# chronista-club/fleetflow

Hardware: AMD Instinct MI355X
Metric: container x node evaluations/sec (FFD what-if plans, work-equivalent) + achieved GB/s % HBM roofline (higher is better)
Workload: dtype u32

## Files before the change

### fleetflow_amd/csrc/fp_internal.h

```cpp
#pragma once
#include <cmath>
#include <cstring>
#include <hip/hip_runtime.h>
#include <stdint.h>
#include <vector>
#include "../../include/fleetplace.h"
#include "fp_rows.h"

#define FP_HIP(call)                                   \
    do {                                               \
        hipError_t e_ = (call);                        \
        if (e_ != hipSuccess) return fp_hip_fail(e_);  \
    } while (0)

int fp_hip_fail(hipError_t e);

__device__ __forceinline__ void fp_or_new_bits(uint32_t *w, uint32_t bits) {
    if (bits & ~*(volatile uint32_t *)w) atomicOr(w, bits);
}

struct fp_ctx {
    int device = 0;
    hipStream_t own_stream = nullptr;
    hipStream_t stream = nullptr;
// ... 115 lines not shown
    const double r = pow((double)hi / (double)lo, 1.0 / (double)(FP_BUCKETS - 2));
    double v = (double)lo;
    for (int k = 1; k < FP_BUCKETS; ++k) {
        uint32_t x = k == FP_BUCKETS - 1 ? hi : (uint32_t)ceil(v);
        if (x < T[k - 1]) x = T[k - 1];
        if (x > hi) x = hi;
        T[k] = x;
        v *= r;
    }
}
struct fp_pipe_soa {
    uint32_t *s_cpu, *s_mem, *s_req, *s_conf, *s_idx;
};
int fp_pipe_soa_take(fp_ctx *c, size_t SC, fp_pipe_soa *soa);
uint32_t fp_pipe_kpack(const fp_ctx *c, uint32_t C);
int fp_pipe_launch(fp_ctx *c, uint32_t S, uint32_t C, uint32_t N, uint32_t scen_base, const uint32_t *order,
                   const void *skeys, uint32_t key_bytes, uint32_t mbits, uint64_t cmax, uint64_t mmax,
                   const uint32_t *cval, const uint32_t *mval, const fp_batch *b, const uint32_t *thr,
                   const fp_pipe_soa *ready, uint32_t *rng);

namespace fpd {

constexpr uint64_t GAMMA = 0x9E3779B97F4A7C15ull;
constexpr uint64_t TAG_CONT = 0xC0C0C0C0C0C0C0C0ull;
constexpr uint64_t TAG_NODE = 0x5E5E5E5E5E5E5E5Eull;

__host__ __device__ inline uint64_t draw(uint64_t seed, uint64_t idx) {
    uint64_t z = seed + (idx + 1) * GAMMA;
    z = (z ^ (z >> 30)) * 0xBF58476D1CE4E5B9ull;
    z = (z ^ (z >> 27)) * 0x94D049BB133111EBull;
    return z ^ (z >> 31);
// ... 18 lines not shown
```

### fleetflow_amd/csrc/fp_pipe.hip

```cpp
#include "fp_internal.h"
#include "fp_pipe_asm.h"
#include "fp_pipe_sys.h"
#include "fp_pipe_pk.h"
#include "fp_pipe_tus.h"
#include <stdlib.h>
#include <string.h>
#include <mutex>
#include <type_traits>
#include <utility>

#ifdef FP_PIPE_STATS
__device__ unsigned long long g_pipe_stats[16 * 16];
#define STAT_ADD(w, i, v) atomicAdd(&g_pipe_stats[(w) * 16 + (i)], (unsigned long long)(v))
#define STAT_CLK() __builtin_amdgcn_s_memtime()
#define STAT_ON 1
#ifdef FP_PIPE_STATS_FINE
#define STAT_GCLK() __builtin_amdgcn_s_memtime()
#define STAT_FINE 1
#else
#define STAT_GCLK() 0ull
#define STAT_FINE 0
#endif
constexpr int TL_B = 2048;
__device__ unsigned long long g_pipe_tl[16 * TL_B * 8];
// ... 33 lines not shown
    uint32_t flush;
    uint32_t kpack;
    uint32_t publish;
    uint32_t pub_mask;
    uint32_t sys;
    uint32_t *ticket;
    uint32_t *gabort;
    uint32_t *ghead;
    uint32_t *gdata;
    uint32_t *part;
    const uint32_t *s_cpu, *s_mem, *s_req, *s_conf, *s_idx;
    uint32_t *cf, *mf;
    const uint32_t *lab;
    uint32_t *cu;
    const uint8_t *sched;
    uint32_t *assign;
    uint8_t *reason;
    uint64_t *cost;
    uint32_t *err;
    uint64_t spin_ticks;
    const uint32_t *thr;
    uint32_t prio;
    uint32_t *rng;
    uint32_t pk_mode;
};

__device__ __forceinline__ uint32_t lds_acq(uint32_t *p) {
    return __builtin_amdgcn_readfirstlane(__hip_atomic_load(p, __ATOMIC_ACQUIRE, __HIP_MEMORY_SCOPE_WORKGROUP));
}
__device__ __forceinline__ void lds_rel(uint32_t *p, uint32_t v) {
    __hip_atomic_store(p, v, __ATOMIC_RELEASE, __HIP_MEMORY_SCOPE_WORKGROUP);
}

__device__ __forceinline__ uint32_t g_ld(const uint32_t *p) {
    return __hip_atomic_load(const_cast<uint32_t *>(p), __ATOMIC_RELAXED, __HIP_MEMORY_SCOPE_AGENT);
}
__device__ __forceinline__ uint32_t g_ld_u(const uint32_t *p) {
    return __builtin_amdgcn_readfirstlane(g_ld(p));
}
__device__ __forceinline__ void g_st(uint32_t *p, uint32_t v) {
// ... 501 lines not shown
                req = valid ? nf_req : 0u;
                conf = valid ? nf_conf : 0u;
                idx = valid ? nf_idx : 0u;
            } else {
                if (valid) {
                    cpu = a.s_cpu[cb + i];
                    mem = a.s_mem[cb + i];
                    req = a.s_req[cb + i];
                    conf = a.s_conf[cb + i];
                    idx = a.s_idx[cb + i];
                }
                if constexpr (DB) __builtin_amdgcn_s_waitcnt(VMCNT0);
            }
            const bool cyc = valid && (idx & CYC);
            if (cyc) {
                const uint32_t j = idx & pmask;
                a.assign[cb + j] = FP_NONE;
                a.reason[cb + j] = (uint8_t)req;
            }
            n_rej += (uint32_t)__popcll(__ballot(cyc));
            valid = valid && !cyc;
            k0 += 64;
            if constexpr (LA >= 2) {
                if (k0 < C) {
                    const size_t ti = cb + min(k0 + (lane == 0 ? 0u : lane == 1 ? 32u : 63u), C - 1);
                    g_touch(a.s_cpu + ti);
                    g_touch(a.s_mem + ti);
                    g_touch(a.s_req + ti);
                    g_touch(a.s_conf + ti);
                    g_touch(a.s_idx + ti);
                }
            }
        } else {
// ... 123 lines not shown
#ifdef FP_PIPE_STATS
        const unsigned long long tl_cand = ck_b;
        const uint32_t tl_idx = st_batches - 1;
#endif
        if constexpr (DB_EARLY) {
            asm volatile("" : "+v"(nf_cpu), "+v"(nf_mem), "+v"(nf_req), "+v"(nf_conf), "+v"(nf_idx), "+v"(la2_n),
                         "+v"(la2_pos));
            if (g_in) {
                nf_idx = la_pos;
                la_n = la2_n;
                la_pos = la2_pos;
            }
        } else if constexpr (DB) {
            FPP_REQUEST_NEXT();
        }
        if ((placed >> lane) & 1ull) a.assign[cb + (idx & pmask)] = my_assign;
#ifdef FP_PIPE_STATS
        if (s == 0 && lane == 0 && tl_idx < (uint32_t)TL_B && b * W + w < 16) {
            unsigned long long *tl = &g_pipe_tl[((size_t)(b * W + w) * TL_B + tl_idx) * 8];
            tl[0] = tl_top; tl[1] = tl_avail; tl[2] = ck_t0_batch; tl[3] = tl_pre; tl[4] = tl_cand;
            tl[5] = st_checks - tl_checks0; tl[6] = st_hits - tl_hits0;
            tl[7] = tl_todo | ((unsigned long long)__popcll(vm) << 32);
        }
#endif
        const bool fwd = valid && !((placed >> lane) & 1ull);
        if (g_out) {
            const uint64_t fm = __builtin_amdgcn_ballot_w64(fwd);
            const uint32_t f = (uint32_t)__popcll(fm);
            if (f) {
                const uint32_t pos = ofill + fpp_rank(fm);
                if (gbounded &&
// ... 18 lines not shown
                    ofill += f;
                }
            }
            if (tail_issued && ofill && __builtin_amdgcn_readfirstlane(tail_async) + 1u >= ohead) {
                if (lane == 0) g_st(gout_data + (size_t)GSLOT(ohead) * LSLOT, ofill);
                asm volatile("s_waitcnt vmcnt(0)" ::: "memory");
                ohead++;
                if (lane == 0) g_st(gout_head, ohead);
                ofill = 0;
                opend = 0;
            }
            if (STAT_FINE) { ck_b = STAT_GCLK(); ck_fwd += ck_b - ck_a; }
            continue;
        }
        if (!has_out) {
            if (fwd) {
                a.assign[cb + (idx & pmask)] = FP_NONE;
                a.reason[cb + (idx & pmask)] = FP_REASON_NOFIT;
            }
            n_rej += (uint32_t)__popcll(__ballot(fwd));
            continue;
        }
        const uint64_t fm = __ballot(fwd);
        const uint32_t f = (uint32_t)__popcll(fm);
        if (f) {
            const uint32_t pos = ofill + fpp_rank(fm);
            uint32_t *od = odata + (size_t)(ohead % R) * NF * 64;
            if (fwd && pos < 64) {
                od[pos] = cpu; od[64 + pos] = mem; od[128 + pos] = req; od[192 + pos] = conf; od[256 + pos] = idx;
            }
            if (ofill + f >= 64) {
                octl[2 + ohead % R] = 64;
                ohead++;
                lds_rel(&octl[0], ohead);
// ... 255 lines not shown
#pragma unroll
        for (int u = 0; u < 4; ++u) {
            const size_t i = i0 + (size_t)u * stride;
            if (i < total) {
                __builtin_nontemporal_store(cv[u], &s_cpu[i]);
                __builtin_nontemporal_store(mv[u], &s_mem[i]);
                __builtin_nontemporal_store(r[u], &s_req[i]);
                __builtin_nontemporal_store(f[u], &s_conf[i]);
                const uint32_t kb = kpack ? (bucket(T, cv[u]) << 21) | (bucket(T + K, mv[u]) << 26) : 0u;
                __builtin_nontemporal_store(pos[u] | kb | cy[u], &s_idx[i]);
            }
        }
    }
}

__global__ void k_gather_payload(uint32_t S, uint32_t C, const uint32_t *__restrict__ order,
                                 const uint32_t *__restrict__ req, const uint32_t *__restrict__ conf,
                                 const uint32_t *__restrict__ level, const uint32_t *__restrict__ summ,
                                 uint32_t *__restrict__ s_req, uint32_t *__restrict__ s_conf,
                                 uint32_t *__restrict__ s_idx) {
    const uint32_t total = S * C;
    const uint32_t lb = (gridDim.x & 7u) ? blockIdx.x : (blockIdx.x & 7u) * (gridDim.x >> 3) + (blockIdx.x >> 3);
    const uint32_t i0 = lb * 4 * blockDim.x + threadIdx.x;
    uint32_t src[4], r[4], f[4], cy[4];
#pragma unroll
    for (int u = 0; u < 4; ++u) {
        const uint32_t i = i0 + u * blockDim.x;
        if (i < total) src[u] = i - i % C + __builtin_nontemporal_load(&order[i]);
    }
#pragma unroll
    for (int u = 0; u < 4; ++u) {
        const uint32_t i = i0 + u * blockDim.x;
        if (i < total) {
            r[u] = req[src[u]];
            f[u] = conf[src[u]];
            cy[u] = (level && level[src[u]] == FP_NONE) ? CYC : 0u;
            if (cy[u]) {
                r[u] = FP_REASON_CYCLE;
            } else if (summ && screened(summ + (size_t)(i / C) * 4, r[u], f[u])) {
                cy[u] = CYC;
                r[u] = FP_REASON_NOFIT;
            }
        }
    }
#pragma unroll
    for (int u = 0; u < 4; ++u) {
        const uint32_t i = i0 + u * blockDim.x;
        if (i < total) {
            __builtin_nontemporal_store(r[u], &s_req[i]);
            __builtin_nontemporal_store(f[u], &s_conf[i]);
            if (cy[u]) s_idx[i] |= CYC;
        }
    }
}

constexpr uint32_t PL_THREADS = 1024, PL_H = 25, PL_MAX_C = PL_THREADS * PL_H * 2;
constexpr uint32_t PL_CHUNK = 18 * 1024;
__global__ __launch_bounds__(1024) void k_payload_lds(uint32_t C, const uint32_t *__restrict__ order,
                                                      const uint32_t *__restrict__ req,
                                                      const uint32_t *__restrict__ conf,
                                                      const uint32_t *__restrict__ level,
                                                      const uint32_t *__restrict__ summ,
                                                      uint32_t *__restrict__ s_req, uint32_t *__restrict__ s_conf,
                                                      uint32_t *__restrict__ s_idx) {
    extern __shared__ uint2 pl_lds2[];
    uint32_t *pl_lds = reinterpret_cast<uint32_t *>(pl_lds2);
    const uint32_t t = threadIdx.x;
    const size_t cb = (size_t)blockIdx.x * C;
    const uint32_t sm0 = summ ? summ[(size_t)blockIdx.x * 4] : 0xFFFFFFFFu;
    const uint32_t sm1 = summ ? summ[(size_t)blockIdx.x * 4 + 1] : 0u;
    for (uint32_t h = 0; h < 2; ++h) {
        const uint32_t pbase = h * PL_THREADS * PL_H + t;
        if (h * PL_THREADS * PL_H >= C) break;
        uint32_t o[PL_H];
#pragma unroll
        for (uint32_t j = 0; j < PL_H; ++j) {
            const uint32_t p = pbase + PL_THREADS * j;
            o[j] = p < C ? __builtin_nontemporal_load(&order[cb + p]) : 0xFFFFFFFFu;
        }
        uint32_t vr[PL_H], vf[PL_H];
        uint32_t cy = 0;
        if (level) {
            for (uint32_t a0 = 0; a0 < C; a0 += 2 * PL_CHUNK) {
                const uint32_t n = C - a0 < 2 * PL_CHUNK ? C - a0 : 2 * PL_CHUNK;
                __syncthreads();
#pragma unroll 4
                for (uint32_t i = t; i < n; i += PL_THREADS) pl_lds[i] = __builtin_nontemporal_load(&level[cb + a0 + i]);
                __syncthreads();
#pragma unroll
                for (uint32_t j = 0; j < PL_H; ++j) {
                    const uint32_t d = o[j] - a0;
                    if (d < n) cy |= (uint32_t)(pl_lds[d] == FP_NONE) << j;
                }
// ... 18 lines not shown
            if (p < C) {
                uint32_t r = vr[j];
                const bool c = (cy >> j) & 1u, x = ((r & ~sm0) | (vf[j] & sm1)) != 0u;
                if (c) r = FP_REASON_CYCLE;
                else if (summ && x) r = FP_REASON_NOFIT;
                __builtin_nontemporal_store(r, &s_req[cb + p]);
                __builtin_nontemporal_store(vf[j], &s_conf[cb + p]);
                if (c || (summ && x)) s_idx[cb + p] |= CYC;
            }
        }
    }
}

constexpr uint32_t UNSORT_SPAN16 = 50 * 1024;
constexpr uint32_t UNSORT_SPAN32 = 30 * 1024;
template <bool NARROW>
__global__ __launch_bounds__(1024) void k_unsort(uint32_t C, uint32_t H, uint32_t span,
                                                 const uint32_t *__restrict__ order,
                                                 const uint32_t *__restrict__ asg_s, const uint8_t *__restrict__ rsn_s,
                                                 uint32_t *__restrict__ assign, uint8_t *__restrict__ reason) {
    using A = typename std::conditional<NARROW, uint16_t, uint32_t>::type;
    extern __shared__ __attribute__((aligned(16))) unsigned char ulds[];
    A *la = reinterpret_cast<A *>(ulds);
    uint8_t *lr = ulds + (size_t)span * sizeof(A);
    const uint32_t s = blockIdx.x / H, h = blockIdx.x % H;
    const uint32_t lo = h * span, hi = min(C, lo + span);
    const size_t cb = (size_t)s * C;
    constexpr uint32_t U = 8;
    for (uint32_t p0 = threadIdx.x; p0 < C; p0 += blockDim.x * U) {
        uint32_t j[U], av[U];
        uint8_t rv[U];
#pragma unroll
        for (uint32_t u = 0; u < U; ++u) {
            const uint32_t p = p0 + u * blockDim.x;
            j[u] = p < C ? __builtin_nontemporal_load(&order[cb + p]) : 0xFFFFFFFFu;
            av[u] = p < C ? __builtin_nontemporal_load(&asg_s[cb + p]) : 0u;
            rv[u] = p < C ? __builtin_nontemporal_load(&rsn_s[cb + p]) : 0;
        }
#pragma unroll
        for (uint32_t u = 0; u < U; ++u) {
            if (j[u] >= lo && j[u] < hi) {
                la[j[u] - lo] = (A)av[u];
                lr[j[u] - lo] = av[u] != FP_NONE ? (uint8_t)FP_REASON_OK : rv[u];
            }
        }
    }
    __syncthreads();
    for (uint32_t j = lo + threadIdx.x; j < hi; j += blockDim.x) {
        const A v = la[j - lo];
        __builtin_nontemporal_store(NARROW && v == (A)0xFFFF ? FP_NONE : (uint32_t)v, &assign[cb + j]);
        reason[cb + j] = lr[j - lo];
    }
}

size_t lds_bytes(uint32_t W, uint32_t G, uint32_t R) {
    return (size_t)W * G * K * 16 + ((size_t)(W - 1) * 8 + 8) * 4 + (size_t)(W - 1) * R * NF * 64 * 4;
}

template <uint32_t G, uint32_t BLK = 1024, uint32_t WV = 0, bool PK = false>
static int launch_g(hipStream_t st, unsigned grid, unsigned block, size_t lds, const PipeArgs &a) {
    if (block > BLK) return FP_EINVAL;
    FP_HIP(hipFuncSetAttribute((const void *)k_ffd_pipe<G, BLK, WV, PK>, hipFuncAttributeMaxDynamicSharedMemorySize,
                               (int)lds));
    k_ffd_pipe<G, BLK, WV, PK><<<grid, block, lds, st>>>(a);
    return FP_OK;
}

// ... 221 lines not shown
        const int64_t sv = fp_opt(c, FP_OPT_SYSTOLIC_VALU, 2);
        if (sv == 1) g->sys_extra |= 0x8000u;
        else if (sv == 2) g->sys_extra |= 0x4000u;
    }
    {
        const int64_t pv = fp_opt(c, FP_OPT_PIPE_PRIO, wide12_big(S, W, G) ? 0 : 1);
        g->prio = pv >= 0 && pv <= 2 ? (uint32_t)pv : 0u;
    }
    return true;
}

size_t fp_pipe_ws_bytes(fp_ctx *c, uint32_t S, uint32_t C, uint32_t N) {
    PipeGeom g;
    if (!pipe_geom(c, S, C, N, &g)) return 0;
    const size_t SC = (size_t)S * C, nlinks = (size_t)S * (g.B - 1);
    return 5 * SC * 4 + SC * 5 + 256 + nlinks * LCTL * 4 + (size_t)S * g.B * 8 + 8 + nlinks * g.slots * 2 * 64 * 4 +
           (size_t)S * 16 + 11 * 256;
}

uint32_t fp_pipe_kpack(const fp_ctx *c, uint32_t C) {
    return C <= (IDX_POS_MASK + 1u) && fp_opt(c, FP_OPT_KPACK, 1) != 0;
}

int fp_pipe_soa_take(fp_ctx *c, size_t SC, fp_pipe_soa *soa) {
    soa->s_cpu = (uint32_t *)fp_ws_take(c, SC * 4);
    soa->s_mem = (uint32_t *)fp_ws_take(c, SC * 4);
    soa->s_req = (uint32_t *)fp_ws_take(c, SC * 4);
    soa->s_conf = (uint32_t *)fp_ws_take(c, SC * 4);
    soa->s_idx = (uint32_t *)fp_ws_take(c, SC * 4);
    return (soa->s_cpu && soa->s_mem && soa->s_req && soa->s_conf && soa->s_idx) ? FP_OK : FP_ENOMEM;
}

int fp_pipe_launch(fp_ctx *c, uint32_t S, uint32_t C, uint32_t N, uint32_t scen_base, const uint32_t *order,
                   const void *skeys, uint32_t key_bytes, uint32_t mbits, uint64_t cmax, uint64_t mmax,
                   const uint32_t *cval, const uint32_t *mval, const fp_batch *b, const uint32_t *thr,
                   const fp_pipe_soa *ready, uint32_t *rng) {
    PipeGeom geo;
    if (!pipe_geom(c, S, C, N, &geo)) return FP_EOVERFLOW;
    const uint32_t G = geo.G, W = geo.W, B = geo.B, R = geo.R, slots = geo.slots;
    const size_t lds = geo.lds;
    if (C >= 0x80000000u) return FP_EOVERFLOW;
    if ((uint64_t)S * B > 0xFFFFFFFFull) return FP_EOVERFLOW;
    hipStream_t st = c->stream;
    const size_t SC = (size_t)S * C;
    const size_t nlinks = (size_t)S * (B - 1);
    fp_pipe_soa soa;
    if (ready) soa = *ready;
    else if (int rc0 = fp_pipe_soa_take(c, SC, &soa)) return rc0;
    uint32_t *s_cpu = soa.s_cpu, *s_mem = soa.s_mem, *s_req = soa.s_req, *s_conf = soa.s_conf, *s_idx = soa.s_idx;
    uint32_t *ctl = (uint32_t *)fp_ws_take(c, 256 + nlinks * LCTL * 4);
    uint32_t *part = (uint32_t *)fp_ws_take(c, (size_t)S * B * 8 + 8);
    uint32_t *gdata = nlinks ? (uint32_t *)fp_ws_take(c, nlinks * slots * 2 * 64 * 4) : nullptr;
    uint32_t *asg_s = (uint32_t *)fp_ws_take(c, SC * 4);
    uint8_t *rsn_s = (uint8_t *)fp_ws_take(c, SC);
    if (!ctl || !part || (nlinks && !gdata) || !asg_s || !rsn_s) return FP_ENOMEM;
    FP_HIP(hipMemsetAsync(ctl, 0, 256 + nlinks * LCTL * 4, st));
    const uint32_t kpack = fp_pipe_kpack(c, C);
    uint32_t *summ = nullptr;
    if (N && fp_opt(c, FP_OPT_SCREEN, 1)) {
        summ = (uint32_t *)fp_ws_take(c, (size_t)S * 16);
        if (!summ) return FP_ENOMEM;
    }
    launch_fn u32fn = nullptr, pkfn = nullptr;
    const bool big = wide12_big(S, W, G) && !geo.bounded;
    {
        const void *k_;
        pipe_kernel(G, W, big, false, &u32fn, &k_);
        if (rng && fp_opt(c, FP_OPT_PACKED, 1) != 0) pipe_kernel(G, W, big, true, &pkfn, &k_);
        if (!u32fn) return FP_EOVERFLOW;
    }
    if (N && (summ || pkfn)) {
        if (summ && pkfn) k_node_summary<true, true><<<S, 256, 0, st>>>(N, b->cpu_free, b->mem_free, b->labels, b->conflict_used, b->schedulable, summ, rng);
        else if (summ) k_node_summary<true, false><<<S, 256, 0, st>>>(N, b->cpu_free, b->mem_free, b->labels, b->conflict_used, b->schedulable, summ, rng);
        else k_node_summary<false, true><<<S, 256, 0, st>>>(N, b->cpu_free, b->mem_free, b->labels, b->conflict_used, b->schedulable, summ, rng);
        FP_HIP(hipGetLastError());
    }
    const int64_t pl_mode = fp_opt(c, FP_OPT_PAYLOAD_LDS, 1);
    if (ready && C && C <= PL_MAX_C && pl_mode != 0) {
        const size_t pl = (size_t)PL_CHUNK * 8;
        FP_HIP(hipFuncSetAttribute((const void *)k_payload_lds, hipFuncAttributeMaxDynamicSharedMemorySize, (int)pl));
        k_payload_lds<<<S, PL_THREADS, pl, st>>>(C, order, b->req_labels, b->conflict, b->level, summ, s_req, s_conf,
                                                 s_idx);
        FP_HIP(hipGetLastError());
    } else if (ready) {
        size_t g = (SC + 1023) / 1024;
        if (g >= 64) g = (g + 7) & ~(size_t)7;
        k_gather_payload<<<(unsigned)g, 256, 0, st>>>(S, C, order, b->req_labels, b->conflict, b->level, summ,
                                                      s_req, s_conf, s_idx);
        FP_HIP(hipGetLastError());
    } else {
        size_t g = (SC + 1023) / 1024;
        if (g >= 64) g = (g + 7) & ~(size_t)7;
        if (key_bytes == 4)
            k_gather_sorted<uint32_t><<<(unsigned)g, 256, 0, st>>>(
                thr, kpack, S, C, order, (const uint32_t *)skeys, mbits, cmax, mmax, cval, mval, b->cpu_m, b->mem_mib, b->req_labels,
                b->conflict, b->level, summ, s_cpu, s_mem, s_req, s_conf, s_idx);
        else
            k_gather_sorted<uint64_t><<<(unsigned)g, 256, 0, st>>>(
                thr, kpack, S, C, order, (const uint64_t *)skeys, mbits, cmax, mmax, cval, mval, b->cpu_m, b->mem_mib, b->req_labels,
                b->conflict, b->level, summ, s_cpu, s_mem, s_req, s_conf, s_idx);
        FP_HIP(hipGetLastError());
    }
    PipeArgs a;
    a.C = C; a.N = N; a.scen_base = scen_base; a.W = W; a.G = G; a.R = R;
    a.B = B; a.slots = slots; a.bounded = geo.bounded; a.ticket = ctl; a.gabort = ctl + 32; a.ghead = ctl + 64;
    a.gdata = gdata;
    a.S = S;
    a.lag = geo.lag;
    a.kpack = kpack;
    a.flush = (geo.bounded ? 3u : 1u) & (uint32_t)fp_opt(c, FP_OPT_PIPE_FLUSH, 3);
    a.part = part;
    a.s_cpu = s_cpu; a.s_mem = s_mem; a.s_req = s_req; a.s_conf = s_conf; a.s_idx = s_idx;
    a.cf = b->cpu_free; a.mf = b->mem_free; a.lab = b->labels; a.cu = b->conflict_used; a.sched = b->schedulable;
    a.assign = asg_s; a.reason = rsn_s; a.cost = b->cost; a.err = c->d_err;
    a.spin_ticks = (uint64_t)fp_opt(c, FP_OPT_SPIN_TICKS, (int64_t)SPIN_TICKS);
    a.sys = geo.sys ? (geo.sys | (geo.sys_extra << 16)) : 0u;
    {
        const int64_t pv = fp_opt(c, FP_OPT_LINK_PUBLISH, S >= 4096 ? 32 : 8);
        a.publish = geo.bounded ? 1u : (uint32_t)(pv < 1 ? 1 : pv > 1024 ? 1024 : pv);
        uint32_t p2 = 1;
        while (p2 * 2 <= a.publish) p2 *= 2;
        a.pub_mask = p2 - 1;
    }
    a.thr = thr;
    a.prio = geo.prio;
    const bool wide = wide_g(W, G);
    if (G < 1 || (wide ? (G > MAX_G_WIDE || G % 4) : G > MAX_G)) return FP_EOVERFLOW;
    std::unique_lock<std::mutex> gate_lock;
    BoundedGate *gate = nullptr;
// ... 16 lines not shown
            a.pk_mode = 2;
            rc = pkfn(st, (unsigned)(S * B), W * 64, lds, a);
        }
    } else {
        a.pk_mode = 0;
        rc = u32fn(st, (unsigned)(S * B), W * 64, lds, a);
    }
    if (rc) return rc;
    FP_HIP(hipGetLastError());
    fp_prof_end(c, FP_K_PLACE, ev);
    if (gate) {
        FP_HIP(hipEventRecord(gate->ev, st));
        gate_lock.unlock();
    }
    {
        const bool narrow16 = N < 0xFFFFu;
        const uint32_t span = narrow16 ? UNSORT_SPAN16 : UNSORT_SPAN32;
        const uint32_t H = (C + span - 1) / span;
        const size_t ul = (size_t)span * (narrow16 ? 3 : 5);
        const void *fn = narrow16 ? (const void *)k_unsort<true> : (const void *)k_unsort<false>;
        FP_HIP(hipFuncSetAttribute(fn, hipFuncAttributeMaxDynamicSharedMemorySize, (int)ul));
        if (narrow16)
            k_unsort<true><<<(unsigned)(S * H), 1024, ul, st>>>(C, H, span, order, asg_s, rsn_s, b->assign, b->reason);
        else
            k_unsort<false><<<(unsigned)(S * H), 1024, ul, st>>>(C, H, span, order, asg_s, rsn_s, b->assign, b->reason);
        FP_HIP(hipGetLastError());
    }
    if (b->cost) {
        k_cost_reduce<<<(S + 255) / 256, 256, 0, st>>>(S, B, scen_base, part, b->cost);
        FP_HIP(hipGetLastError());
    }
    return FP_OK;
}

int fp_place_geometry_impl(fp_ctx *c, uint32_t S, uint32_t C, uint32_t N, uint32_t *out) {
    PipeGeom g;
    if (!pipe_geom(c, S, C, N, &g)) return FP_EOVERFLOW;
    const uint32_t v[FP_GEOM_COUNT] = {g.G, g.W, g.B, g.R, g.lag, g.slots, g.bounded, g.resident, g.sys};
    memcpy(out, v, sizeof(v));
    return FP_OK;
}
// ... 54 lines not shown
```

### fleetflow_amd/csrc/fp_place.hip

```cpp
#include "fp_internal.h"

namespace {

__device__ __forceinline__ void bounds_acc(uint32_t c, uint32_t m, uint32_t &mc, uint32_t &mm, uint32_t &lc,
                                           uint32_t &lm) {
    mc = max(mc, c);
    mm = max(mm, m);
    lc = c ? min(lc, c) : lc;
    lm = m ? min(lm, m) : lm;
}


constexpr uint32_t RANK_MAX_VALUE = 1u << 18;
constexpr uint32_t RANK_WORDS = RANK_MAX_VALUE / 32;

enum { CN_DC = 0, CN_DM = 1, CN_OVER = 6, CN_MAXC = 8, CN_MAXM = 9, CN_MINC = 10, CN_MINM = 11, CN_ORC = 12, CN_ORM = 13,
       CN_WORDS = 16 };
__global__ __launch_bounds__(256) void k_value_bitmap(const uint32_t *__restrict__ cpu,
                                                      const uint32_t *__restrict__ mem, size_t n,
                                                      uint32_t *__restrict__ gbc, uint32_t *__restrict__ gbm,
                                                      uint32_t *__restrict__ cnt) {
    extern __shared__ uint32_t lbm[];
    for (uint32_t i = threadIdx.x; i < 2 * RANK_WORDS; i += blockDim.x) lbm[i] = 0;
    __syncthreads();
// ... 136 lines not shown
constexpr size_t SR_BYTES = (size_t)SR_W * (4 + 2) * 2;
constexpr size_t SS_TAB_BYTES = SS_DIG * (4 + 4 + 1 + 1);
constexpr size_t SS_IMG_BYTES = SR_BYTES + SS_TAB_BYTES;

__host__ __device__ static inline size_t ss_align16(size_t b) { return (b + 15) & ~(size_t)15; }
__host__ __device__ static inline size_t ss_xr_bytes(uint32_t C) {
    return ss_align16((size_t)C * 2 > SR_BYTES ? (size_t)C * 2 : SR_BYTES);
}
static inline size_t ss_lds_bytes(uint32_t C) {
    return ss_xr_bytes(C) + ss_align16(C) + SS_WAVES * SS_DIG * 2 + 2 * SS_DIG * 4 + 2 * SS_DIG * 4 + 2 * SS_DIG + 16;
}

struct ScenSortArgs {
    uint32_t C, kpack;
    const uint32_t *cpu, *mem;
    uint32_t *order, *s_cpu, *s_mem, *s_idx;
    const uint32_t *T;
    const uint32_t *scnt;
    const unsigned char *simg;
    uint32_t *rng;
};

typedef uint64_t __attribute__((may_alias)) ss_u64a;
typedef uint32_t __attribute__((may_alias)) ss_u32a;
typedef uint32_t ss_u32x4 __attribute__((ext_vector_type(4)));

__device__ __forceinline__ uint64_t ss_match(uint32_t v, bool valid, uint32_t nb) {
    uint64_t m = __builtin_amdgcn_ballot_w64(valid);
    for (uint32_t b = 0; b < nb; ++b) {
        const bool bit = (v >> b) & 1u;
        const uint64_t bb = __builtin_amdgcn_ballot_w64(bit);
// ... 60 lines not shown
            WH[ww * SS_DIG + t] = (uint16_t)run;
            run += c;
        }
        HB[t] = run;
    }
    __syncthreads();
}

__device__ void ss_generic(const ScenSortArgs &a, uint16_t *X, uint16_t *WH, uint32_t *HS, uint32_t *HB,
                           size_t cb, uint32_t C) {
    const uint32_t t = threadIdx.x, lane = t & 63, w = t >> 6;
    const uint64_t lt = (1ull << lane) - 1ull;
    const uint32_t L = (C + SS_WAVES - 1) / SS_WAVES;
    const uint32_t s0 = min(C, w * L), s1 = min(C, s0 + L);
    uint16_t *myrow = WH + w * SS_DIG;
    uint32_t *ord = a.order + cb;
    const uint32_t *cpu = a.cpu + cb, *mem = a.mem + cb;
    for (uint32_t k = 0; k < 8; ++k) {
        const uint32_t *key = k < 4 ? mem : cpu;
        const uint32_t sh = 8u * (k & 3u);
        auto src = [&](uint32_t p) -> uint32_t {
            return k == 0 ? p
                   : (k & 1u) ? (uint32_t)X[p]
                              : __hip_atomic_load(&ord[p], __ATOMIC_RELAXED, __HIP_MEMORY_SCOPE_AGENT);
        };
        for (uint32_t i = t; i < SS_WAVES * SS_DIG / 2; i += blockDim.x) reinterpret_cast<ss_u32a *>(WH)[i] = 0u;
        __syncthreads();
        for (uint32_t p = s0 + lane; p < s1; p += 64) ss_inc16(myrow, ((~key[src(p)]) >> sh) & 0xFFu);
        __syncthreads();
        ss_offsets(WH, HS, HB, t, lane, w);
        for (uint32_t p0 = s0; p0 < s1; p0 += 64) {
            const uint32_t p = p0 + lane;
            const bool valid = p < s1;
            const uint32_t j = valid ? src(p) : 0u;
            const uint32_t d = valid ? ((~key[j]) >> sh) & 0xFFu : 0u;
            const uint64_t m = ss_match(d, valid, 8);
            const uint32_t off = myrow[d];
            __builtin_amdgcn_fence(__ATOMIC_SEQ_CST, "wavefront");
            if (valid) {
                if ((m & lt) == 0) myrow[d] = (uint16_t)(off + __popcll(m));
                const uint32_t q = off + (uint32_t)__popcll(m & lt);
                if (k & 1u) ord[q] = j;
                else X[q] = (uint16_t)j;
            }
            __builtin_amdgcn_fence(__ATOMIC_SEQ_CST, "wavefront");
        }
        __syncthreads();
    }
    uint32_t oc = 0, om = 0;
    for (uint32_t P = t; P < C; P += blockDim.x) {
        const uint32_t j = __hip_atomic_load(&ord[P], __ATOMIC_RELAXED, __HIP_MEMORY_SCOPE_AGENT);
        const uint32_t cv = cpu[j], mv = mem[j];
        a.s_cpu[cb + P] = cv;
        a.s_mem[cb + P] = mv;
        a.s_idx[cb + P] = P | (a.kpack ? (ss_bucket(a.T, cv) << 21) | (ss_bucket(a.T + FP_BUCKETS, mv) << 26) : 0u);
        oc |= cv;
        om |= mv;
// ... 275 lines not shown
            __builtin_amdgcn_fence(__ATOMIC_SEQ_CST, "workgroup");
#pragma unroll
            for (uint32_t k = 0; k < SS_REG; ++k) {
                if (lo + 64 * k >= hi) break;
                const bool valid = lo + 64 * k + lane < hi;
                const uint64_t m = ss_match(lv[k], valid, lbits);
                const uint32_t off = myrow[lv[k]];
                if (valid) {
                    if ((m & lt) == 0) myrow[lv[k]] = (uint16_t)(off + __popcll(m));
                    X[off + (uint32_t)__popcll(m & lt)] = (uint16_t)jv[k];
                }
            }
            __builtin_amdgcn_fence(__ATOMIC_SEQ_CST, "workgroup");
            for (uint32_t P = lo + lane; P < hi; P += 64) {
                const uint32_t j = X[P], l = LD[j];
                a.order[cb + P] = j;
                a.s_cpu[cb + P] = cv;
                a.s_mem[cb + P] = MV[l];
                a.s_idx[cb + P] = P | kbc | (a.kpack ? (uint32_t)MB[l] << 26 : 0u);
            }
        } else {
#pragma unroll 4
            for (uint32_t p = lo + lane; p < hi; p += 64) ss_inc16(myrow, LD[X[p]]);
            __builtin_amdgcn_fence(__ATOMIC_SEQ_CST, "workgroup");
            ss_row_scan(myrow, lane, lo);
            __builtin_amdgcn_fence(__ATOMIC_SEQ_CST, "workgroup");
            for (uint32_t p0 = lo; p0 < hi; p0 += 64) {
                const uint32_t p = p0 + lane;
                const bool valid = p < hi;
                const uint32_t j = valid ? X[p] : 0u;
                const uint32_t l = valid ? LD[j] : 0u;
                const uint64_t m = ss_match(l, valid, lbits);
                const uint32_t off = myrow[l];
                if (valid) {
                    if ((m & lt) == 0) myrow[l] = (uint16_t)(off + __popcll(m));
                    const uint32_t P = off + (uint32_t)__popcll(m & lt);
                    a.order[cb + P] = j;
                    a.s_cpu[cb + P] = cv;
                    a.s_mem[cb + P] = MV[l];
                    a.s_idx[cb + P] = P | kbc | (a.kpack ? (uint32_t)MB[l] << 26 : 0u);
                }
            }
        }
        __builtin_amdgcn_fence(__ATOMIC_SEQ_CST, "workgroup");
    }
#ifdef FP_PIPE_STATS
    const unsigned long long ck4 = SS_CLK();
    if (lane == 0) {
        atomicAdd(&g_sort_stats[4], ck4 - ck3);
        atomicMax(&g_sort_stats[6], (unsigned long long)big);
    }
    __syncthreads();
// ... 86 lines not shown
    return FP_OK;
}
#endif

constexpr uint32_t THR_SAMPLE = 8;

static int place_ws_need(fp_ctx *c, uint32_t S, uint32_t C, uint32_t N, size_t *need, fp_ffd_order *fo) {
    if (int rc = fp_ffd_order_size(c, S, C, 0, fo)) return rc;
    const size_t pipe_ws = fp_pipe_ws_bytes(c, S, C, N);
    if (pipe_ws == 0) return FP_EOVERFLOW;
    const size_t rank_ws = 2 * (2 * RANK_WORDS * 4 + RANK_MAX_VALUE * 4) + CN_WORDS * 4 + 2 * FP_BUCKETS * 4 + 3 * 256
                           + SS_IMG_BYTES + 256;
    *need = rank_ws + fo->bytes + pipe_ws + 2 * 256;
    return FP_OK;
}

int fp_place_ws_bytes_impl(fp_ctx *c, uint32_t S, uint32_t C, uint32_t N, uint64_t *bytes) {
    if (S == 0 || C == 0) { *bytes = 0; return FP_OK; }
    if ((size_t)S * C > 0xFFFFFFFFull) return FP_EOVERFLOW;
    size_t need = 0;
    fp_ffd_order fo;
    if (int rc = place_ws_need(c, S, C, N, &need, &fo)) return rc;
    *bytes = need;
    return FP_OK;
}

int fp_dev_place_batch_impl(fp_ctx *c, const fp_batch *b) {
    const uint32_t S = b->n_scen, C = b->n_containers, N = b->n_nodes;
    c->last_rng = nullptr;
    if (S == 0) return FP_OK;
// ... 41 lines not shown
                                   (int)(2 * RANK_WORDS * 4)));
        k_value_bitmap<<<gb, 256, 2 * RANK_WORDS * 4, st>>>(b->cpu_m, b->mem_mib, n, rbm, rbm + RANK_WORDS, rcnt);
        FP_HIP(hipGetLastError());
        k_rank_tables<<<2, 1024, 0, st>>>(rbm, rbm + RANK_WORDS, RANK_WORDS, RANK_WORDS, rpre, rpre + RANK_WORDS, rval,
                                          rval + RANK_MAX_VALUE, rcnt);
        FP_HIP(hipGetLastError());
        k_thresholds<<<1, 64, 0, st>>>(rcnt, rval, rval + RANK_MAX_VALUE, thr);
        FP_HIP(hipGetLastError());
    }
    if (ss_lds_bytes(C) <= SS_LDS_CAP && C <= SS_WAVES * SS_CHUNKS * 64 && fp_opt(c, FP_OPT_SCEN_SORT, 1) != 0) {
        ScenSortArgs sa;
        sa.C = C; sa.kpack = fp_pipe_kpack(c, C);
        sa.cpu = b->cpu_m; sa.mem = b->mem_mib;
        fp_pipe_soa soa;
        if (int rs = fp_pipe_soa_take(c, SC, &soa)) return rs;
        uint32_t *order = (uint32_t *)fp_ws_take(c, SC * 4);
        if (!order) return FP_ENOMEM;
        sa.order = order; sa.s_cpu = soa.s_cpu; sa.s_mem = soa.s_mem; sa.s_idx = soa.s_idx;
        sa.T = thr;
        sa.scnt = rcnt;
        sa.rng = rcnt + CN_ORC;
        sa.simg = simg;
        k_sort_image<<<1, 1024, 0, st>>>(rbm, rpre, rval, rcnt, thr, sa.kpack, simg);
        FP_HIP(hipGetLastError());
        const size_t lds = ss_lds_bytes(C);
        FP_HIP(hipFuncSetAttribute((const void *)k_scen_sort, hipFuncAttributeMaxDynamicSharedMemorySize, (int)lds));
        k_scen_sort<<<S, 1024, lds, st>>>(sa);
        FP_HIP(hipGetLastError());
        fp_prof_end(c, FP_K_SORT, ev);
        return fp_pipe_launch(c, S, C, N, b->scen_base, order, nullptr, 4, 0, 0, 0, rval, rval + RANK_MAX_VALUE, b,
                              thr, &soa, rcnt + CN_ORC);
    }
    const uint64_t full = 0xFFFFFFFFull;
    if (int rs = fp_ffd_order_run(c, S, C, b->cpu_m, b->mem_mib, rcnt + CN_ORC, &fo)) return rs;
    fp_prof_end(c, FP_K_SORT, ev);
    return fp_pipe_launch(c, S, C, N, b->scen_base, fo.order, fo.keys_out, 8, 32, full, full, nullptr, nullptr, b, thr,
                          nullptr, rcnt + CN_ORC);
}

extern "C" int fp_ctx_place_path(fp_ctx *c, uint32_t *out3) {
    if (!c || !out3) return FP_EINVAL;
    out3[0] = out3[1] = out3[2] = 0u;
    if (!c->last_rng) return FP_OK;
    FP_HIP(hipSetDevice(c->device));
    FP_HIP(hipStreamSynchronize(c->stream));
    FP_HIP(hipMemcpy(out3, c->last_rng, 12, hipMemcpyDeviceToHost));
    return FP_OK;
}

extern "C" int fp_dev_argmin_cost(fp_ctx *c, const uint64_t *cost, uint32_t n, uint32_t *best) {
    if (!c || !cost || !best || n == 0) return FP_EINVAL;
    FP_HIP(hipSetDevice(c->device));
// ... 4 lines not shown
```

Before: 72780 billion.

## Narrow sort order to u16 and merge assign/reason into one compact result word

The scenario-sort path now writes the per-scenario order permutation as 16-bit indices, and every downstream consumer (payload gather, LDS payload, unsort) reads them at that width. The pipeline's separate 32-bit assign and 8-bit reason scratch arrays become a single result array, 16-bit when N fits, with reason codes encoded as sentinel values near the top of the range. Unsort decodes that array back into assign and reason. This cuts scratch traffic and LDS use in the placement and unsort stages, at the cost of extra decode logic and a new dependence on C fitting in 16 bits for the sorted path. A post-launch check that the workspace stayed within its computed size is also added.

```diff
diff --git a/fleetflow_amd/csrc/fp_internal.h b/fleetflow_amd/csrc/fp_internal.h
--- a/fleetflow_amd/csrc/fp_internal.h
+++ b/fleetflow_amd/csrc/fp_internal.h
@@ -153,7 +153,7 @@
 };
 int fp_pipe_soa_take(fp_ctx *c, size_t SC, fp_pipe_soa *soa);
 uint32_t fp_pipe_kpack(const fp_ctx *c, uint32_t C);
-int fp_pipe_launch(fp_ctx *c, uint32_t S, uint32_t C, uint32_t N, uint32_t scen_base, const uint32_t *order,
+int fp_pipe_launch(fp_ctx *c, uint32_t S, uint32_t C, uint32_t N, uint32_t scen_base, const void *order,
                    const void *skeys, uint32_t key_bytes, uint32_t mbits, uint64_t cmax, uint64_t mmax,
                    const uint32_t *cval, const uint32_t *mval, const fp_batch *b, const uint32_t *thr,
                    const fp_pipe_soa *ready, uint32_t *rng);
diff --git a/fleetflow_amd/csrc/fp_pipe.hip b/fleetflow_amd/csrc/fp_pipe.hip
--- a/fleetflow_amd/csrc/fp_pipe.hip
+++ b/fleetflow_amd/csrc/fp_pipe.hip
@@ -71,8 +71,8 @@
     const uint32_t *lab;
     uint32_t *cu;
     const uint8_t *sched;
-    uint32_t *assign;
-    uint8_t *reason;
+    void *res;
+    uint32_t res16;
     uint64_t *cost;
     uint32_t *err;
     uint64_t spin_ticks;
@@ -81,6 +81,17 @@
     uint32_t *rng;
     uint32_t pk_mode;
 };
+
+constexpr uint32_t RES_NOFIT = 0u - (uint32_t)FP_REASON_NOFIT, RES_CYCLE = 0u - (uint32_t)FP_REASON_CYCLE;
+static_assert(RES_NOFIT == FP_NONE && RES_CYCLE == FP_NONE - 1u, "result sentinels");
+constexpr uint32_t RES16_MAX_N = 0xFFFEu;
+static inline size_t res_word_bytes(uint32_t N) { return N <= RES16_MAX_N ? 2 : 4; }
+
+__device__ __forceinline__ void res_store(const PipeArgs &a, size_t cb, uint32_t pos, uint32_t v) {
+    char *row16 = reinterpret_cast<char *>(a.res) + (cb << 1);
+    if (a.res16) *reinterpret_cast<uint16_t *>(row16 + (uint32_t)(pos << 1)) = (uint16_t)v;
+    else reinterpret_cast<uint32_t *>(a.res)[cb + pos] = v;
+}
 
 __device__ __forceinline__ uint32_t lds_acq(uint32_t *p) {
     return __builtin_amdgcn_readfirstlane(__hip_atomic_load(p, __ATOMIC_ACQUIRE, __HIP_MEMORY_SCOPE_WORKGROUP));
@@ -612,9 +623,7 @@
             }
             const bool cyc = valid && (idx & CYC);
             if (cyc) {
-                const uint32_t j = idx & pmask;
-                a.assign[cb + j] = FP_NONE;
-                a.reason[cb + j] = (uint8_t)req;
+                res_store(a, cb, idx & pmask, 0u - req);
             }
             n_rej += (uint32_t)__popcll(__ballot(cyc));
             valid = valid && !cyc;
@@ -768,7 +777,7 @@
         } else if constexpr (DB) {
             FPP_REQUEST_NEXT();
         }
-        if ((placed >> lane) & 1ull) a.assign[cb + (idx & pmask)] = my_assign;
+        if ((placed >> lane) & 1ull) res_store(a, cb, idx & pmask, my_assign);
 #ifdef FP_PIPE_STATS
         if (s == 0 && lane == 0 && tl_idx < (uint32_t)TL_B && b * W + w < 16) {
             unsigned long long *tl = &g_pipe_tl[((size_t)(b * W + w) * TL_B + tl_idx) * 8];
@@ -817,10 +826,7 @@
             continue;
         }
         if (!has_out) {
-            if (fwd) {
-                a.assign[cb + (idx & pmask)] = FP_NONE;
-                a.reason[cb + (idx & pmask)] = FP_REASON_NOFIT;
-            }
+            if (fwd) res_store(a, cb, idx & pmask, RES_NOFIT);
             n_rej += (uint32_t)__popcll(__ballot(fwd));
             continue;
         }
@@ -1106,7 +1112,7 @@
     }
 }
 
-__global__ void k_gather_payload(uint32_t S, uint32_t C, const uint32_t *__restrict__ order,
+__global__ void k_gather_payload(uint32_t S, uint32_t C, const uint16_t *__restrict__ order,
                                  const uint32_t *__restrict__ req, const uint32_t *__restrict__ conf,
                                  const uint32_t *__restrict__ level, const uint32_t *__restrict__ summ,
                                  uint32_t *__restrict__ s_req, uint32_t *__restrict__ s_conf,
@@ -1118,7 +1124,7 @@
 #pragma unroll
     for (int u = 0; u < 4; ++u) {
         const uint32_t i = i0 + u * blockDim.x;
-        if (i < total) src[u] = i - i % C + __builtin_nontemporal_load(&order[i]);
+        if (i < total) src[u] = i - i % C + (uint32_t)__builtin_nontemporal_load(&order[i]);
     }
 #pragma unroll
     for (int u = 0; u < 4; ++u) {
@@ -1148,7 +1154,7 @@
 
 constexpr uint32_t PL_THREADS = 1024, PL_H = 25, PL_MAX_C = PL_THREADS * PL_H * 2;
 constexpr uint32_t PL_CHUNK = 18 * 1024;
-__global__ __launch_bounds__(1024) void k_payload_lds(uint32_t C, const uint32_t *__restrict__ order,
+__global__ __launch_bounds__(1024) void k_payload_lds(uint32_t C, const uint16_t *__restrict__ order,
                                                       const uint32_t *__restrict__ req,
                                                       const uint32_t *__restrict__ conf,
                                                       const uint32_t *__restrict__ level,
@@ -1168,7 +1174,7 @@
 #pragma unroll
         for (uint32_t j = 0; j < PL_H; ++j) {
             const uint32_t p = pbase + PL_THREADS * j;
-            o[j] = p < C ? __builtin_nontemporal_load(&order[cb + p]) : 0xFFFFFFFFu;
+            o[j] = p < C ? (uint32_t)__builtin_nontemporal_load(&order[cb + p]) : 0xFFFFFFFFu;
         }
         uint32_t vr[PL_H], vf[PL_H];
         uint32_t cy = 0;
@@ -1217,43 +1223,48 @@
 
 constexpr uint32_t UNSORT_SPAN16 = 50 * 1024;
 constexpr uint32_t UNSORT_SPAN32 = 30 * 1024;
-template <bool NARROW>
-__global__ __launch_bounds__(1024) void k_unsort(uint32_t C, uint32_t H, uint32_t span,
-                                                 const uint32_t *__restrict__ order,
-                                                 const uint32_t *__restrict__ asg_s, const uint8_t *__restrict__ rsn_s,
-                                                 uint32_t *__restrict__ assign, uint8_t *__restrict__ reason) {
-    using A = typename std::conditional<NARROW, uint16_t, uint32_t>::type;
+template <class A, class O>
+__global__ __launch_bounds__(1024) void k_unsort(uint32_t C, uint32_t H, uint32_t span, const O *__restrict__ order,
+                                                 const A *__restrict__ res, uint32_t *__restrict__ assign,
+                                                 uint8_t *__restrict__ reason) {
     extern __shared__ __attribute__((aligned(16))) unsigned char ulds[];
     A *la = reinterpret_cast<A *>(ulds);
-    uint8_t *lr = ulds + (size_t)span * sizeof(A);
     const uint32_t s = blockIdx.x / H, h = blockIdx.x % H;
     const uint32_t lo = h * span, hi = min(C, lo + span);
     const size_t cb = (size_t)s * C;
     constexpr uint32_t U = 8;
     for (uint32_t p0 = threadIdx.x; p0 < C; p0 += blockDim.x * U) {
-        uint32_t j[U], av[U];
-        uint8_t rv[U];
+        uint32_t j[U];
+        A av[U];
 #pragma unroll
         for (uint32_t u = 0; u < U; ++u) {
             const uint32_t p = p0 + u * blockDim.x;
-            j[u] = p < C ? __builtin_nontemporal_load(&order[cb + p]) : 0xFFFFFFFFu;
-            av[u] = p < C ? __builtin_nontemporal_load(&asg_s[cb + p]) : 0u;
-            rv[u] = p < C ? __builtin_nontemporal_load(&rsn_s[cb + p]) : 0;
-        }
-#pragma unroll
-        for (uint32_t u = 0; u < U; ++u) {
-            if (j[u] >= lo && j[u] < hi) {
-                la[j[u] - lo] = (A)av[u];
-                lr[j[u] - lo] = av[u] != FP_NONE ? (uint8_t)FP_REASON_OK : rv[u];
-            }
-        }
+            j[u] = p < C ? (uint32_t)__builtin_nontemporal_load(&order[cb + p]) : 0xFFFFFFFFu;
+            av[u] = p < C ? __builtin_nontemporal_load(&res[cb + p]) : (A)0;
+        }
+#pragma unroll
+        for (uint32_t u = 0; u < U; ++u)
+            if (j[u] >= lo && j[u] < hi) la[j[u] - lo] = av[u];
     }
     __syncthreads();
     for (uint32_t j = lo + threadIdx.x; j < hi; j += blockDim.x) {
         const A v = la[j - lo];
-        __builtin_nontemporal_store(NARROW && v == (A)0xFFFF ? FP_NONE : (uint32_t)v, &assign[cb + j]);
-        reason[cb + j] = lr[j - lo];
-    }
+        const bool none = v >= (A)RES_CYCLE;
+        __builtin_nontemporal_store(none ? FP_NONE : (uint32_t)v, &assign[cb + j]);
+        reason[cb + j] = none ? (uint8_t)((A)0 - v) : (uint8_t)FP_REASON_OK;
+    }
+}
+
+template <class A, class O>
+static int launch_unsort(hipStream_t st, uint32_t S, uint32_t C, const void *order, const void *res, uint32_t *assign,
+                         uint8_t *reason) {
+    const uint32_t span = sizeof(A) == 2 ? UNSORT_SPAN16 : UNSORT_SPAN32;
+    const uint32_t H = (C + span - 1) / span;
+    const size_t ul = (size_t)span * sizeof(A);
+    FP_HIP(hipFuncSetAttribute((const void *)k_unsort<A, O>, hipFuncAttributeMaxDynamicSharedMemorySize, (int)ul));
+    k_unsort<A, O><<<(unsigned)(S * H), 1024, ul, st>>>(C, H, span, (const O *)order, (const A *)res, assign, reason);
+    FP_HIP(hipGetLastError());
+    return FP_OK;
 }
 
 size_t lds_bytes(uint32_t W, uint32_t G, uint32_t R) {
@@ -1505,8 +1516,8 @@
     PipeGeom g;
     if (!pipe_geom(c, S, C, N, &g)) return 0;
     const size_t SC = (size_t)S * C, nlinks = (size_t)S * (g.B - 1);
-    return 5 * SC * 4 + SC * 5 + 256 + nlinks * LCTL * 4 + (size_t)S * g.B * 8 + 8 + nlinks * g.slots * 2 * 64 * 4 +
-           (size_t)S * 16 + 11 * 256;
+    return 5 * SC * 4 + SC * res_word_bytes(N) + 256 + nlinks * LCTL * 4 + (size_t)S * g.B * 8 + 8 +
+           nlinks * g.slots * 2 * 64 * 4 + (size_t)S * 16 + 10 * 256;
 }
 
 uint32_t fp_pipe_kpack(const fp_ctx *c, uint32_t C) {
@@ -1522,7 +1533,7 @@
     return (soa->s_cpu && soa->s_mem && soa->s_req && soa->s_conf && soa->s_idx) ? FP_OK : FP_ENOMEM;
 }
 
-int fp_pipe_launch(fp_ctx *c, uint32_t S, uint32_t C, uint32_t N, uint32_t scen_base, const uint32_t *order,
+int fp_pipe_launch(fp_ctx *c, uint32_t S, uint32_t C, uint32_t N, uint32_t scen_base, const void *order,
                    const void *skeys, uint32_t key_bytes, uint32_t mbits, uint64_t cmax, uint64_t mmax,
                    const uint32_t *cval, const uint32_t *mval, const fp_batch *b, const uint32_t *thr,
                    const fp_pipe_soa *ready, uint32_t *rng) {
@@ -1542,9 +1553,9 @@
     uint32_t *ctl = (uint32_t *)fp_ws_take(c, 256 + nlinks * LCTL * 4);
     uint32_t *part = (uint32_t *)fp_ws_take(c, (size_t)S * B * 8 + 8);
     uint32_t *gdata = nlinks ? (uint32_t *)fp_ws_take(c, nlinks * slots * 2 * 64 * 4) : nullptr;
-    uint32_t *asg_s = (uint32_t *)fp_ws_take(c, SC * 4);
-    uint8_t *rsn_s = (uint8_t *)fp_ws_take(c, SC);
-    if (!ctl || !part || (nlinks && !gdata) || !asg_s || !rsn_s) return FP_ENOMEM;
+    const uint32_t res16 = res_word_bytes(N) == 2;
+    void *res = fp_ws_take(c, SC * res_word_bytes(N));
+    if (!ctl || !part || (nlinks && !gdata) || !res) return FP_ENOMEM;
     FP_HIP(hipMemsetAsync(ctl, 0, 256 + nlinks * LCTL * 4, st));
     const uint32_t kpack = fp_pipe_kpack(c, C);
     uint32_t *summ = nullptr;
@@ -1570,25 +1581,26 @@
     if (ready && C && C <= PL_MAX_C && pl_mode != 0) {
         const size_t pl = (size_t)PL_CHUNK * 8;
         FP_HIP(hipFuncSetAttribute((const void *)k_payload_lds, hipFuncAttributeMaxDynamicSharedMemorySize, (int)pl));
-        k_payload_lds<<<S, PL_THREADS, pl, st>>>(C, order, b->req_labels, b->conflict, b->level, summ, s_req, s_conf,
-                                                 s_idx);
+        k_payload_lds<<<S, PL_THREADS, pl, st>>>(C, (const uint16_t *)order, b->req_labels, b->conflict, b->level, summ,
+                                                 s_req, s_conf, s_idx);
         FP_HIP(hipGetLastError());
     } else if (ready) {
         size_t g = (SC + 1023) / 1024;
         if (g >= 64) g = (g + 7) & ~(size_t)7;
-        k_gather_payload<<<(unsigned)g, 256, 0, st>>>(S, C, order, b->req_labels, b->conflict, b->level, summ,
-                                                      s_req, s_conf, s_idx);
+        k_gather_payload<<<(unsigned)g, 256, 0, st>>>(S, C, (const uint16_t *)order, b->req_labels, b->conflict, b->level,
+                                                      summ, s_req, s_conf, s_idx);
         FP_HIP(hipGetLastError());
     } else {
         size_t g = (SC + 1023) / 1024;
         if (g >= 64) g = (g + 7) & ~(size_t)7;
+        const uint32_t *order32 = (const uint32_t *)order;
         if (key_bytes == 4)
             k_gather_sorted<uint32_t><<<(unsigned)g, 256, 0, st>>>(
-                thr, kpack, S, C, order, (const uint32_t *)skeys, mbits, cmax, mmax, cval, mval, b->cpu_m, b->mem_mib, b->req_labels,
+                thr, kpack, S, C, order32, (const uint32_t *)skeys, mbits, cmax, mmax, cval, mval, b->cpu_m, b->mem_mib, b->req_labels,
                 b->conflict, b->level, summ, s_cpu, s_mem, s_req, s_conf, s_idx);
         else
             k_gather_sorted<uint64_t><<<(unsigned)g, 256, 0, st>>>(
-                thr, kpack, S, C, order, (const uint64_t *)skeys, mbits, cmax, mmax, cval, mval, b->cpu_m, b->mem_mib, b->req_labels,
+                thr, kpack, S, C, order32, (const uint64_t *)skeys, mbits, cmax, mmax, cval, mval, b->cpu_m, b->mem_mib, b->req_labels,
                 b->conflict, b->level, summ, s_cpu, s_mem, s_req, s_conf, s_idx);
         FP_HIP(hipGetLastError());
     }
@@ -1603,7 +1615,7 @@
     a.part = part;
     a.s_cpu = s_cpu; a.s_mem = s_mem; a.s_req = s_req; a.s_conf = s_conf; a.s_idx = s_idx;
     a.cf = b->cpu_free; a.mf = b->mem_free; a.lab = b->labels; a.cu = b->conflict_used; a.sched = b->schedulable;
-    a.assign = asg_s; a.reason = rsn_s; a.cost = b->cost; a.err = c->d_err;
+    a.res = res; a.res16 = res16; a.cost = b->cost; a.err = c->d_err;
     a.spin_ticks = (uint64_t)fp_opt(c, FP_OPT_SPIN_TICKS, (int64_t)SPIN_TICKS);
     a.sys = geo.sys ? (geo.sys | (geo.sys_extra << 16)) : 0u;
     {
@@ -1650,17 +1662,9 @@
         gate_lock.unlock();
     }
     {
-        const bool narrow16 = N < 0xFFFFu;
-        const uint32_t span = narrow16 ? UNSORT_SPAN16 : UNSORT_SPAN32;
-        const uint32_t H = (C + span - 1) / span;
-        const size_t ul = (size_t)span * (narrow16 ? 3 : 5);
-        const void *fn = narrow16 ? (const void *)k_unsort<true> : (const void *)k_unsort<false>;
-        FP_HIP(hipFuncSetAttribute(fn, hipFuncAttributeMaxDynamicSharedMemorySize, (int)ul));
-        if (narrow16)
-            k_unsort<true><<<(unsigned)(S * H), 1024, ul, st>>>(C, H, span, order, asg_s, rsn_s, b->assign, b->reason);
-        else
-            k_unsort<false><<<(unsigned)(S * H), 1024, ul, st>>>(C, H, span, order, asg_s, rsn_s, b->assign, b->reason);
-        FP_HIP(hipGetLastError());
+        const auto unsort = res16 ? (ready ? launch_unsort<uint16_t, uint16_t> : launch_unsort<uint16_t, uint32_t>)
+                                  : (ready ? launch_unsort<uint32_t, uint16_t> : launch_unsort<uint32_t, uint32_t>);
+        if (int ru = unsort(st, S, C, order, res, b->assign, b->reason)) return ru;
     }
     if (b->cost) {
         k_cost_reduce<<<(S + 255) / 256, 256, 0, st>>>(S, B, scen_base, part, b->cost);
diff --git a/fleetflow_amd/csrc/fp_place.hip b/fleetflow_amd/csrc/fp_place.hip
--- a/fleetflow_amd/csrc/fp_place.hip
+++ b/fleetflow_amd/csrc/fp_place.hip
@@ -174,7 +174,8 @@
 struct ScenSortArgs {
     uint32_t C, kpack;
     const uint32_t *cpu, *mem;
-    uint32_t *order, *s_cpu, *s_mem, *s_idx;
+    uint16_t *order;
+    uint32_t *s_cpu, *s_mem, *s_idx;
     const uint32_t *T;
     const uint32_t *scnt;
     const unsigned char *simg;
@@ -265,7 +266,7 @@
     const uint32_t L = (C + SS_WAVES - 1) / SS_WAVES;
     const uint32_t s0 = min(C, w * L), s1 = min(C, s0 + L);
     uint16_t *myrow = WH + w * SS_DIG;
-    uint32_t *ord = a.order + cb;
+    uint16_t *ord = a.order + cb;
     const uint32_t *cpu = a.cpu + cb, *mem = a.mem + cb;
     for (uint32_t k = 0; k < 8; ++k) {
         const uint32_t *key = k < 4 ? mem : cpu;
@@ -273,7 +274,7 @@
         auto src = [&](uint32_t p) -> uint32_t {
             return k == 0 ? p
                    : (k & 1u) ? (uint32_t)X[p]
-                              : __hip_atomic_load(&ord[p], __ATOMIC_RELAXED, __HIP_MEMORY_SCOPE_AGENT);
+                              : (uint32_t)__hip_atomic_load(&ord[p], __ATOMIC_RELAXED, __HIP_MEMORY_SCOPE_AGENT);
         };
         for (uint32_t i = t; i < SS_WAVES * SS_DIG / 2; i += blockDim.x) reinterpret_cast<ss_u32a *>(WH)[i] = 0u;
         __syncthreads();
@@ -291,7 +292,7 @@
             if (valid) {
                 if ((m & lt) == 0) myrow[d] = (uint16_t)(off + __popcll(m));
                 const uint32_t q = off + (uint32_t)__popcll(m & lt);
-                if (k & 1u) ord[q] = j;
+                if (k & 1u) ord[q] = (uint16_t)j;
                 else X[q] = (uint16_t)j;
             }
             __builtin_amdgcn_fence(__ATOMIC_SEQ_CST, "wavefront");
@@ -597,7 +598,7 @@
             __builtin_amdgcn_fence(__ATOMIC_SEQ_CST, "workgroup");
             for (uint32_t P = lo + lane; P < hi; P += 64) {
                 const uint32_t j = X[P], l = LD[j];
-                a.order[cb + P] = j;
+                a.order[cb + P] = (uint16_t)j;
                 a.s_cpu[cb + P] = cv;
                 a.s_mem[cb + P] = MV[l];
                 a.s_idx[cb + P] = P | kbc | (a.kpack ? (uint32_t)MB[l] << 26 : 0u);
@@ -618,7 +619,7 @@
                 if (valid) {
                     if ((m & lt) == 0) myrow[l] = (uint16_t)(off + __popcll(m));
                     const uint32_t P = off + (uint32_t)__popcll(m & lt);
-                    a.order[cb + P] = j;
+                    a.order[cb + P] = (uint16_t)j;
                     a.s_cpu[cb + P] = cv;
                     a.s_mem[cb + P] = MV[l];
                     a.s_idx[cb + P] = P | kbc | (a.kpack ? (uint32_t)MB[l] << 26 : 0u);
@@ -735,6 +736,8 @@
     *need = rank_ws + fo->bytes + pipe_ws + 2 * 256;
     return FP_OK;
 }
+
+static int ws_within(const fp_ctx *c, size_t need, int rc) { return rc == FP_OK && c->ws_top > need ? FP_ENOMEM : rc; }
 
 int fp_place_ws_bytes_impl(fp_ctx *c, uint32_t S, uint32_t C, uint32_t N, uint64_t *bytes) {
     if (S == 0 || C == 0) { *bytes = 0; return FP_OK; }
@@ -806,7 +809,7 @@
         sa.cpu = b->cpu_m; sa.mem = b->mem_mib;
         fp_pipe_soa soa;
         if (int rs = fp_pipe_soa_take(c, SC, &soa)) return rs;
-        uint32_t *order = (uint32_t *)fp_ws_take(c, SC * 4);
+        uint16_t *order = (uint16_t *)fp_ws_take(c, SC * 2);
         if (!order) return FP_ENOMEM;
         sa.order = order; sa.s_cpu = soa.s_cpu; sa.s_mem = soa.s_mem; sa.s_idx = soa.s_idx;
         sa.T = thr;
@@ -820,14 +823,14 @@
         k_scen_sort<<<S, 1024, lds, st>>>(sa);
         FP_HIP(hipGetLastError());
         fp_prof_end(c, FP_K_SORT, ev);
-        return fp_pipe_launch(c, S, C, N, b->scen_base, order, nullptr, 4, 0, 0, 0, rval, rval + RANK_MAX_VALUE, b,
-                              thr, &soa, rcnt + CN_ORC);
+        return ws_within(c, need, fp_pipe_launch(c, S, C, N, b->scen_base, order, nullptr, 4, 0, 0, 0, rval,
+                                                 rval + RANK_MAX_VALUE, b, thr, &soa, rcnt + CN_ORC));
     }
     const uint64_t full = 0xFFFFFFFFull;
     if (int rs = fp_ffd_order_run(c, S, C, b->cpu_m, b->mem_mib, rcnt + CN_ORC, &fo)) return rs;
     fp_prof_end(c, FP_K_SORT, ev);
-    return fp_pipe_launch(c, S, C, N, b->scen_base, fo.order, fo.keys_out, 8, 32, full, full, nullptr, nullptr, b, thr,
-                          nullptr, rcnt + CN_ORC);
+    return ws_within(c, need, fp_pipe_launch(c, S, C, N, b->scen_base, fo.order, fo.keys_out, 8, 32, full, full, nullptr,
+                                             nullptr, b, thr, nullptr, rcnt + CN_ORC));
 }
 
 extern "C" int fp_ctx_place_path(fp_ctx *c, uint32_t *out3) {
```

Measured after the change: 74010 billion, median of 5. +1.7%, better.
